# ishine/TargetDiarization

Hardware: AMD Instinct MI355X
Metric: real-time factor (audio-sec/wall-sec) full infer() pipe, 16kHz mono, 1/2/4/8 GPU (higher is better)
Workload: dtype f32 (split-f16 x3: fp32-accurate products from three f16 MFMA passes, fp32 accumulate); 1 GPU; BASELINE configs[3]: 1800 s synthetic conversation (two alternating speakers, 20 % overlap) = 180 x 10 s windows: MossFormer2 (90 windows per launch) -> loudness swap -> ERes2NetV2 on every 10 s window of both streams + cosine vs a target embedding -> Paraformer (SANM encoder, CIF predictor, NAR decoder, argmax tokens + timestamps) on 30 s segments of both streams -> CT-Transformer punctuation of ; windows_per_launch=90

## Files before the change

targetdiarization_amd/_lib.py:

```python
from __future__ import annotations

import ctypes as C
import os

HERE = os.path.dirname(os.path.abspath(__file__))
LIB_PATH = os.path.join(HERE, "libtdx.so")


class TdxError(RuntimeError):
    pass


class Mf2Config(C.Structure):
    _fields_ = [("num_blocks", C.c_int32), ("channels", C.c_int32), ("kernel_size", C.c_int32),
                ("num_spks", C.c_int32), ("group_size", C.c_int32), ("reserved", C.c_int32 * 3)]


class MdxConfig(C.Structure):
    _fields_ = [("num_blocks", C.c_int32), ("l", C.c_int32), ("g", C.c_int32), ("k", C.c_int32), ("bn", C.c_int32),
                ("dim_f", C.c_int32), ("dim_t", C.c_int32), ("reserved", C.c_int32)]


class WhisperConfig(C.Structure):
    _fields_ = [("n_mels", C.c_int32), ("n_audio_ctx", C.c_int32), ("d_model", C.c_int32), ("enc_heads", C.c_int32),
# ... 159 lines not shown
    "tdx_pvoc_destroy": (_i, [_vp]),
    "tdx_pvoc_prepare": (_i, [_vp, _i]),
    "tdx_pvoc_workspace_bytes": (_sz, [_vp, _i, _i, _i, C.c_long, C.c_long]),
    "tdx_pvoc_stretch": (_i, [_vp, _fp, _i, C.c_long, _vp, _vp, _vp, _i, C.c_long, _fp, _fp, _fp, _vp, _sz, _vp]),
    "tdx_pvoc_vocode": (_i, [_vp, _fp, _i, _i, _i, _vp, _vp, _vp, _i, _fp, _vp]),
    "tdx_pvoc_istft": (_i, [_vp, _fp, _i, _i, _i, C.c_long, _fp, _vp, _sz, _vp]),
    "tdx_pvoc_eq_match": (_i, [_vp, _fp, C.c_long, _fp, C.c_long, _fp, _i, _i, _i, _fp, _fp, _vp, _vp, _fp, _vp, _sz, _vp]),
    "tdx_resample_sinc_length": (C.c_long, [C.c_long, C.c_double]),
    "tdx_resample_sinc": (_i, [_fp, _i, C.c_long, C.c_double, _fp, C.c_long, _vp]),
    "tdx_spectral_workspace_bytes": (_sz, [_i, _i, _i]),
    "tdx_spectral_laplacian": (_i, [_fp, _i, _i, _i, _vp, _vp, _vp, _sz, _vp]),
    "tdx_symeig_lowest": (_i, [_vp, _i, _i, _vp, _vp, _vp, _sz, _vp]),
    "tdx_fft_workspace_bytes": (_sz, [C.c_long, _i]),
    "tdx_fft_c2c": (_i, [_fp, C.c_long, _i, _i, _fp, _vp, _sz, _vp]),
    "tdx_fft_r2c": (_i, [_fp, C.c_long, _i, _fp, _vp, _sz, _vp]),
    "tdx_fft_c2r": (_i, [_fp, C.c_long, _i, _fp, _vp, _sz, _vp]),
    "tdx_fft_band_mix_workspace_bytes": (_sz, [C.c_long]),
    "tdx_fft_band_mix": (_i, [_fp, _fp, C.c_long, C.POINTER(C.c_long), _fp, _fp, _fp, _fp, _vp, _sz, _vp]),
}


def lib():
    global _lib
    if _lib is None:
        if not os.path.exists(LIB_PATH):
            raise TdxError(f"{LIB_PATH} not found: build it with `python -m targetdiarization_amd.build` "
                           "(hipcc --offload-arch=gfx950).  There is no CPU fallback.")
        import torch
        tl = os.path.join(os.path.dirname(torch.__file__), "lib", "libamdhip64.so")
        if os.path.exists(tl):
            C.CDLL(tl, mode=C.RTLD_GLOBAL)
        l = C.CDLL(LIB_PATH)
        for name, (res, args) in SIGNATURES.items():
            fn = getattr(l, name)
            fn.restype = res
            fn.argtypes = args
        _lib = l
    return _lib


_l = C.c_long


class GemmSeg(C.Structure):
    _fields_ = [("A", _vp), ("B", _vp), ("lda", _l), ("ldb", _l), ("strideA", _l), ("strideB", _l), ("strideA2", _l), ("strideB2", _l),
                ("K", _i), ("zdiv", _i), ("kchunk", _i), ("ktotal", _i)]


class H3Seg(C.Structure):
    _fields_ = [("A", _vp), ("B", _vp), ("sa", _vp), ("sb", _vp), ("lda", _l), ("ldb", _l),
                ("strideA", _l), ("strideB", _l), ("strideA2", _l), ("strideB2", _l),
                ("strideSA", _l), ("strideSB", _l), ("strideSA2", _l), ("strideSB2", _l),
                ("sa_mul", _i), ("sb_mul", _i), ("K", _i), ("zdiv", _i), ("kchunk", _i), ("ktotal", _i), ("segk", _i),
                ("strideSeg", _l), ("a_shift", _i), ("a_period", _i), ("a_zero", _vp)]


DIAG_SIGNATURES = {
    "tdx_diag_last_error": (C.c_char_p, []),
    "tdx_h3_gemm_ex": (_i, [_i] * 4 + [C.POINTER(H3Seg)] * 2 + [_i] * 12 + [_vp, _vp, _l, _l, _i, C.POINTER(_i), _vp]),
    "tdx_h3_gemm_f32a": (_i, [_vp, _l, C.c_float, _vp, _vp, _vp] + [_i] * 8 + [_vp, _l, _i, _vp]),
    "tdx_h3_plan": (_i, [_i] * 5 + [C.POINTER(_i)] * 2),
    "tdx_h3_tile_of_block": (_i, [C.POINTER(_i), _i, _i, _i] + [C.POINTER(_i)] * 3),
    "tdx_h3_split_rows_static": (_i, [_vp, _l, _vp, _l, _i, C.c_float, _vp]),
    "tdx_h3_split_rows_long": (_i, [_vp, _l, _vp, _vp, _l, _i, _vp]),
    "tdx_h3_split_kmajor_ex": (_i, [_vp, _l, _vp, _l, _i, C.c_float, _i, _vp, _vp, _i, _i, _vp]),
    "tdx_h3_split_rows": (_i, [_vp, _l, _vp, _vp, _l, _i, _vp]),
    "tdx_h3_split_kmajor": (_i, [_vp, _l, _vp, _l, _i, C.c_float, _vp]),
    "tdx_h3_gemm_x": (_i, [_i] + [_vp] * 5 + [_i] * 3 + [_vp]),
    "tdx_h3_gemm": (_i, [_vp] * 6 + [_i] * 3 + [_vp]),
    "tdx_h3_gemm_variant": (_i, [_vp] * 6 + [_i] * 4 + [_vp]),
    "tdx_linear_variant": (_i, [_vp, _vp, _i, _i, _i, _vp, _i, _vp]),
    "tdx_linear_epi": (_i, [_vp] * 5 + [_i] * 5 + [_vp]),
    "tdx_gemm_f32": (_i, [_i] * 3 + [C.POINTER(GemmSeg)] * 2 + [_i] * 5 + [_vp, _l, _l, _i, C.POINTER(_i), _vp]),
    "tdx_gemm_f32_conv": (_i, [_vp, _l, _vp] + [_i] * 11 + [_vp, _l, _i, C.POINTER(_i), _vp]),
    "tdx_attn_gate_planes_workspace_bytes": (_sz, [_i, _i, _i]),
    "tdx_attn_gate_planes": (_i, [_vp] * 7 + [_i] * 5 + [_vp] * 5 + [_sz, _vp]),
    "tdx_diag_dft_analysis": (_i, [_i, _i, _l, _l, _l, _i, _vp]),
    "tdx_diag_dft_synthesis": (_i, [_i, _i, _l, _l, _i, _vp]),
    "tdx_diag_loader_bind": (_i, [_vp, _sz] + [_i] * 9 + [_vp, _sz, C.POINTER(_i)]),
    "tdx_test_whisper_noise": (_i, [C.c_ulonglong, C.c_ulonglong, _i, _i, _i, _vp, _vp, _vp]),
    "tdx_test_fft_workspace_bytes": (_sz, [_l, _i, _i]),
    "tdx_test_fft_passes": (_i, [_i, _i]),
    "tdx_test_fft_c2c": (_i, [_vp, _l, _i, _i, _vp, _vp, _sz, _vp, _i]),
    "tdx_fill_bench": (_i, [_i, _vp, _l, _i, _i, _vp, _vp]),
    "tdx_fill_bench2": (_i, [_i, _vp, _i, _i, _i, _vp, _vp]),
    "tdx_fill_bench3": (_i, [_vp, _l, _i, _l, _i, _i, _i, _vp, _vp]),
}
DIAG_PATH = os.path.join(HERE, "libtdx_diag.so")
_diag = None


def diag():
    global _diag
    if _diag is None:
        if not os.path.exists(DIAG_PATH):
            raise TdxError(f"{DIAG_PATH} not found: build it with `python -m targetdiarization_amd.build`")
        lib()
        l = C.CDLL(DIAG_PATH)
        for name, (res, args) in DIAG_SIGNATURES.items():
            fn = getattr(l, name)
            fn.restype = res
            fn.argtypes = args
        _diag = l
    return _diag


def check(status: int):
    if status != 0:
        raise TdxError(f"libtdx status {status}: {lib().tdx_last_error().decode()}")


class HandleGuard:

    def __init__(self, device):
        import threading
        self.device = device
        self.lock = threading.RLock()
        self._event = None
        self._ws = None

    def call(self):
        return _GuardedCall(self)

    def workspace(self, nbytes: int):
        import torch
        nbytes = max(int(nbytes), 16)
        if self._ws is None or self._ws.numel() < nbytes:
            if self._ws is not None and self._event is not None:
                self._event.synchronize()
            self._ws = None
            self._ws = torch.empty(nbytes, dtype=torch.uint8, device=self.device)
        return self._ws


class _GuardedCall:
    def __init__(self, g):
        self.g = g

    def __enter__(self):
        import torch
        g = self.g
        g.lock.acquire()
        try:
            self.stream = torch.cuda.current_stream(g.device)
            self.capturing = torch.cuda.is_current_stream_capturing()
            if g._event is not None and not self.capturing:
                self.stream.wait_event(g._event)
        except BaseException:
            g.lock.release()
            raise
        return g

    def __exit__(self, *exc):
        import torch
        g = self.g
        try:
            if not self.capturing:
                if g._event is None:
                    g._event = torch.cuda.Event()
                g._event.record(self.stream)
        finally:
            g.lock.release()
        return False


class Handle:
# ... 82 lines not shown
```

targetdiarization_amd/csrc/diag.hip:

```cpp
#include <hip/hip_runtime.h>

#include <algorithm>
#include <climits>
#include <initializer_list>
#include <string>

#include "../../include/tdx.h"
#include "../../include/tdx_test.h"
#include "dft_basis.hpp"
#include "epilogues.hpp"
#include "fft.hpp"
#include "gemm_h3f.hpp"
#include "mf2_attention.hpp"
#include "weight_pack.hpp"
#include "whisper_noise.hpp"

using namespace tdx;

namespace {
template <class Act>
int linear_epi(const float* a, const float* w, const float* bias, const float* res, float* out, int M, int Npad, int nreal, int K, hipStream_t st) {
    if (res && nreal < Npad) return linear_f32(a, K, w, M, Npad, K, EpiBiasResN<Act>{bias, res, out, Npad, nreal}, st);
    if (res) return linear_f32(a, K, w, M, Npad, K, EpiBiasRes<Act>{bias, res, out, Npad}, st);
    if (nreal < Npad) return linear_f32(a, K, w, M, Npad, K, EpiBiasActN<Act>{bias, out, Npad, nreal}, st);
    return linear_f32(a, K, w, M, Npad, K, EpiBiasAct<Act>{bias, out, Npad}, st);
}

struct EpiPlainN {
    float* out; long ld, strideZ; int nreal;
    __device__ EpiNone col(int, int) const { return EpiNone{}; }
    __device__ EpiNone row(int, int) const { return EpiNone{}; }
    __device__ void store(int z, int m, int n, float v, EpiNone, EpiNone) const {
        if (n < nreal) out[(long)z * strideZ + (long)m * ld + n] = v;
    }
};
struct EpiPlainPair {
    float* out; long ld, strideZ; int nreal, pair_off;
    __device__ EpiNone col(int, int) const { return EpiNone{}; }
    __device__ EpiNone row(int, int) const { return EpiNone{}; }
    __device__ void store2(int z, int m, int c, float v0, float v1, EpiNone, EpiNone) const {
        if (c < nreal) {
            float* o = out + (long)z * strideZ + (long)m * ld;
            o[c] = v0; o[pair_off + c] = v1;
        }
    }
};

void plan_out(const GemmArgs& g, int* plan) {
    if (plan) { plan[0] = g.map_mode; plan[1] = g.mp; plan[2] = g.gw; plan[3] = g.tiles_m; plan[4] = g.tiles_n; }
}
template <bool PAIRED, bool CONV>
void plan_of(GemmArgs g, int batches, int* plan) {
    plan_gemm<PAIRED, CONV>(g, batches);
    plan_out(g, plan);
}

const char* seg_error(const tdx_gemm_seg& s, bool a_kmajor, bool b_kmajor, int batches) {
    if (!s.A || !s.B) return "null operand";
    if (s.K < 32 || s.K % 32) return "need K >= 32, K % 32 == 0";
    if (s.lda < 1 || s.ldb < 1 || s.lda % 4 || s.ldb % 4) return "need lda % 4 == 0, ldb % 4 == 0";
    if (s.strideA < 0 || s.strideB < 0 || s.strideA2 < 0 || s.strideB2 < 0 || s.strideA % 4 || s.strideB % 4 || s.strideA2 % 4 || s.strideB2 % 4)
        return "need batch strides >= 0 and % 4 == 0 (16-byte loads)";
    if (s.zdiv < 1 || s.kchunk < 0) return "need zdiv >= 1, kchunk >= 0";
    if ((a_kmajor || b_kmajor) && (long)s.ktotal - (long)(std::min(s.zdiv, batches) - 1) * s.kchunk < 1)
        return "need ktotal - z2 * kchunk >= 1 for every z2 of a K-major operand";
    return nullptr;
}
GemmSeg seg_of(const tdx_gemm_seg& s) {
    GemmSeg r = make_seg(s.A, s.lda, s.B, s.ldb, s.K, s.strideA, s.strideB, s.ktotal);
    r.zdiv = s.zdiv; r.strideA2 = s.strideA2; r.strideB2 = s.strideB2; r.kchunk = s.kchunk; r.ktotal = s.ktotal;
    return r;
}
template <bool A_KMAJOR, bool B_KMAJOR, bool PAIRED, bool CONV, class Epi>
int run_gemm_f32(const GemmArgs& g, int batches, Epi e, int* plan, hipStream_t st) {
    plan_of<PAIRED, CONV>(g, batches, plan);
    const hipError_t r = launch_gemm<A_KMAJOR, B_KMAJOR, PAIRED, false, Epi, 0, CONV>(g, batches, e, st);
    return r == hipSuccess ? TDX_OK : tdx::fail_hip(r, __FILE__, __LINE__);
}

H3Seg h3_seg_of(const tdx_h3_seg& s) {
    H3Seg r{};
    r.A = (const unsigned char*)s.A; r.B = (const unsigned char*)s.B; r.sa = s.sa; r.sb = s.sb; r.lda = s.lda; r.ldb = s.ldb;
    r.strideA = s.strideA; r.strideB = s.strideB; r.strideA2 = s.strideA2; r.strideB2 = s.strideB2;
    r.strideSA = s.strideSA; r.strideSB = s.strideSB; r.strideSA2 = s.strideSA2; r.strideSB2 = s.strideSB2;
    r.sa_mul = s.sa_mul; r.sb_mul = s.sb_mul; r.K = s.K; r.zdiv = s.zdiv; r.kchunk = s.kchunk; r.ktotal = s.ktotal;
    r.segk = s.segk; r.strideSeg = s.strideSeg; r.a_shift = s.a_shift; r.a_period = s.a_period; r.a_zero = (const unsigned char*)s.a_zero;
    return r;
}
const char* h3_seg_error(const tdx_h3_seg& s, int form, bool first, int batches) {
    const bool twoseg = form & 4, shift_ok = first && form == 4;
    if (!s.A || !s.B || !s.sa || !s.sb) return "null operand or scale";
    if (s.K < 16 || s.K % 16) return "need K >= 16, K % 16 == 0";
    if (twoseg && s.K < 64) return "TWOSEG needs K >= 64 in both segments";
    if (s.lda < 64 || s.ldb < 64 || s.lda % 16 || s.ldb % 16) return "need lda, ldb >= 64 bytes and % 16 == 0 (16-byte loads)";
    for (long v : {s.strideA, s.strideB, s.strideA2, s.strideB2})
        if (v < 0 || v % 16) return "need operand strides >= 0 and % 16 == 0 (16-byte loads)";
// ... 446 lines not shown
    const long row0 = (long)(blockIdx.x / strips) * rows_per_block;
    const int per_row = seg / 1024;
    const int rows_per_it = 32 / per_row;
    float acc = 0.f;
    for (int it = 0; it < iters; ++it) {
        unsigned char* dst = lds + (it & 3) * 32768;
#pragma unroll
        for (int j = 0; j < 4; ++j) {
            const int i = wave * 4 + j;
            const long r = row0 + ((long)it * rows_per_it + i / per_row) % rows_per_block;
            const unsigned char* g = src + r * pitch + (long)strip * seg + (i % per_row) * 1024 + lane * 16;
            __builtin_amdgcn_global_load_lds((const __attribute__((address_space(1))) void*)g,
                                             (__attribute__((address_space(3))) void*)(dst + i * 1024), 16, 0, 0);
        }
        if ((it & 1) == 1) { asm volatile("s_waitcnt vmcnt(4)" ::: "memory"); __builtin_amdgcn_s_barrier(); }
    }
    asm volatile("s_waitcnt vmcnt(0)" ::: "memory");
    __syncthreads();
    acc += reinterpret_cast<const float*>(lds)[threadIdx.x];
    if (acc == 123.456f) sink[0] = acc;
}
}
extern "C" int tdx_fill_bench3(const void* src, long pitch, int seg, long rows_per_block, int strips, int blocks, int iters, float* sink, void* stream) {
    static bool set = false;
    if (!set) { hipFuncSetAttribute(reinterpret_cast<const void*>(&fill_bench3_kernel), hipFuncAttributeMaxDynamicSharedMemorySize, 131072); set = true; }
    hipLaunchKernelGGL(fill_bench3_kernel, dim3(blocks), dim3(512), 131072, (hipStream_t)stream, (const unsigned char*)src, pitch, seg, rows_per_block, strips, iters, sink);
    return hipGetLastError() == hipSuccess ? TDX_OK : TDX_E_HIP;
}
extern "C" int tdx_fill_bench2(int mode, const void* src, int stride, int blocks, int iters, float* sink, void* stream) {
    static bool set = false;
    if (!set) {
        hipFuncSetAttribute(reinterpret_cast<const void*>(&fill_bench2_kernel<0>), hipFuncAttributeMaxDynamicSharedMemorySize, 131072);
        hipFuncSetAttribute(reinterpret_cast<const void*>(&fill_bench2_kernel<1>), hipFuncAttributeMaxDynamicSharedMemorySize, 131072);
        set = true;
    }
    if (mode == 0) hipLaunchKernelGGL(fill_bench2_kernel<0>, dim3(blocks), dim3(512), 131072, (hipStream_t)stream, (const unsigned char*)src, stride, iters, sink);
    else hipLaunchKernelGGL(fill_bench2_kernel<1>, dim3(blocks), dim3(512), 131072, (hipStream_t)stream, (const unsigned char*)src, stride, iters, sink);
    return hipGetLastError() == hipSuccess ? TDX_OK : TDX_E_HIP;
}
extern "C" int tdx_fill_bench(int mode, const void* src, long bytes_per_block, int blocks, int iters, float* sink, void* stream) {
    static bool set = false;
    if (!set) {
        hipFuncSetAttribute(reinterpret_cast<const void*>(&fill_bench_kernel<0>), hipFuncAttributeMaxDynamicSharedMemorySize, 131072);
        hipFuncSetAttribute(reinterpret_cast<const void*>(&fill_bench_kernel<1>), hipFuncAttributeMaxDynamicSharedMemorySize, 131072);
        set = true;
    }
    if (mode == 0) hipLaunchKernelGGL(fill_bench_kernel<0>, dim3(blocks), dim3(512), 131072, (hipStream_t)stream, (const unsigned char*)src, bytes_per_block, iters, sink);
    else hipLaunchKernelGGL(fill_bench_kernel<1>, dim3(blocks), dim3(512), 131072, (hipStream_t)stream, (const unsigned char*)src, bytes_per_block, iters, sink);
    return hipGetLastError() == hipSuccess ? TDX_OK : TDX_E_HIP;
}

static bool fft_tile_ok(int tile_log2) { return tile_log2 >= tdx::fft::MIN_TILE_LOG2 && tile_log2 <= tdx::fft::MAX_TILE_LOG2; }
extern "C" size_t tdx_test_fft_workspace_bytes(long n, int batch, int tile_log2) {
    if (tdx::fft::size_error(n, batch) || !fft_tile_ok(tile_log2)) return 0;
    return std::max<size_t>(tdx::fft::c2c_ws_floats(n, batch, tile_log2), 64) * sizeof(float);
}
extern "C" int tdx_test_fft_passes(int m, int tile_log2) { return m < 0 || m > 27 || !fft_tile_ok(tile_log2) ? 0 : tdx::fft::passes_of(m, tile_log2); }
extern "C" int tdx_test_fft_c2c(const float* x_dev, long n, int batch, int inverse, float* y_dev, void* ws, size_t ws_bytes, void* stream, int tile_log2) {
    if (!x_dev || !y_dev || !ws || x_dev == y_dev) return tdx::fail(TDX_E_INVALID, "tdx_test_fft_c2c: need x_dev, y_dev, ws, x_dev != y_dev");
    if (const char* e = tdx::fft::size_error(n, batch)) return tdx::fail(TDX_E_INVALID, std::string("tdx_test_fft_c2c: ") + e);
    if (!fft_tile_ok(tile_log2)) return tdx::fail(TDX_E_INVALID, "tdx_test_fft_c2c: need 4 <= tile_log2 <= 12");
    if (ws_bytes < tdx_test_fft_workspace_bytes(n, batch, tile_log2)) return tdx::fail(TDX_E_INVALID, "tdx_test_fft_c2c: workspace too small");
    return tdx::fft::c2c(x_dev, n, batch, inverse != 0, y_dev, (float*)ws, tile_log2, (hipStream_t)stream);
}

namespace {
__global__ __launch_bounds__(256) void whisper_noise_kernel(unsigned long long seed, unsigned long long row_stream, int p, int n0, int count,
                                                             float* __restrict__ g, unsigned* __restrict__ word) {
    const int i = blockIdx.x * 256 + threadIdx.x;
    if (i >= count) return;
    const int n = n0 + i;
    const unsigned w = tdx::wh_noise_words(seed, row_stream, p, n >> 2).w[n & 3];
    word[i] = w;
    g[i] = tdx::wh_gumbel(w);
}
}
extern "C" int tdx_test_whisper_noise(unsigned long long seed, unsigned long long row_stream, int p, int n0, int count, float* g_dev, unsigned* word_dev,
                                      void* stream) {
    if (!g_dev || !word_dev || n0 < 0 || p < 0 || count < 1 || n0 > INT_MAX - count)
        return tdx::fail(TDX_E_INVALID, "tdx_test_whisper_noise: need g_dev, word_dev, n0 >= 0, p >= 0, count >= 1");
    hipLaunchKernelGGL(whisper_noise_kernel, dim3((count + 255) / 256), dim3(256), 0, (hipStream_t)stream, seed, row_stream, p, n0, count, g_dev, word_dev);
    return hipGetLastError() == hipSuccess ? TDX_OK : TDX_E_HIP;
}
```

targetdiarization_amd/csrc/paraformer.hip:

```cpp
#include <hip/hip_runtime.h>

#include <cmath>
#include <string>
#include <vector>

#include "../../include/tdx.h"
#include "gemm.hpp"
#include "gemm_x6.hpp"
#include "gemm_h3.hpp"
#include "shared_kernels.hpp"
#include "tdx_common.hpp"
#include "weight_planes.hpp"
#include "epilogues.hpp"
#include "pf_sanm.hpp"
#include "pf_timestamps.hpp"

using namespace tdx;

namespace {

constexpr int D = 512, DIN = 560, DINP = 576, FFN = 2048, H = 4, DK = 128, KS = 11;
constexpr float PF_LN_EPS = 1e-12f;



__global__ void pf_embed_kernel(const float* __restrict__ feats, const float* __restrict__ embed, PfPrompt pr, int nprompt, float* __restrict__ x, int T) {
    const int t = blockIdx.x, b = blockIdx.y, S = nprompt + T;
    const float pos = (float)(t + 1);
    const float inc = 9.210340371976184f / (float)(DIN / 2 - 1);
    const long row = (long)b * S + t;
    const float* src = t < nprompt ? embed + (long)pr.id[t] * DIN : feats + ((long)b * T + (t - nprompt)) * DIN;
    for (int c = threadIdx.x; c < DINP; c += blockDim.x) {
        float v = 0.f;
        if (c < DIN) {
            const int i = c < DIN / 2 ? c : c - DIN / 2;
            const float ang = __fmul_rn(pos, expf((float)i * (-inc)));
            v = src[c] * 22.627416997969522f + (c < DIN / 2 ? sinf(ang) : cosf(ang));
        }
        x[row * DINP + c] = v;
    }
}

__global__ __launch_bounds__(256) void pf_layernorm_kernel(const float* __restrict__ x, long ld, int C, const float* __restrict__ g,
                                                            const float* __restrict__ b, float* __restrict__ out, long ldo, int Cpad,
                                                            long M, float eps) {
    const long m = (long)blockIdx.x * 4 + (threadIdx.x >> 6);
    if (m >= M) return;
    const int lane = threadIdx.x & 63;
    const float* r = x + m * ld;
    float s = 0.f;
    for (int c = lane; c < C; c += 64) s += r[c];
    const float mean = wave_sum(s) / (float)C;
    float q = 0.f;
    for (int c = lane; c < C; c += 64) { const float d = r[c] - mean; q = fmaf(d, d, q); }
    const float rstd = 1.0f / sqrtf(wave_sum(q) / (float)C + eps);
    float* o = out + m * ldo;
    for (int c = lane; c < Cpad; c += 64) o[c] = c < C ? (r[c] - mean) * rstd * g[c] + b[c] : 0.f;
}

template <int NCH>
__global__ __launch_bounds__(256) void pf_layernorm_planes_kernel_t(const float* __restrict__ x, long ld, int C, const float* __restrict__ g,
                                                                     const float* __restrict__ b, unsigned char* __restrict__ hp,
                                                                     float* __restrict__ hs, int Cpad, long M, float eps) {
    const long m = (long)blockIdx.x * 4 + (threadIdx.x >> 6);
    if (m >= M) return;
    const int lane = threadIdx.x & 63;
    const float* r = x + m * ld;
    if (C == Cpad && (C & 511) == 0 && C / 512 <= NCH && (ld & 3) == 0) {
        const int nc = C / 512;
        float xv[NCH][8];
        float s1 = 0.f;
#pragma unroll
        for (int i = 0; i < NCH; ++i) {
            if (i < nc) {
                const f32x4 a0 = ldg4(r + (lane + 64 * i) * 8), a1 = ldg4(r + (lane + 64 * i) * 8 + 4);
#pragma unroll
                for (int j = 0; j < 4; ++j) { xv[i][j] = a0[j]; xv[i][4 + j] = a1[j]; s1 += a0[j] + a1[j]; }
            }
        }
        const float mean1 = wave_sum(s1) / (float)C;
        float q1 = 0.f;
#pragma unroll
        for (int i = 0; i < NCH; ++i)
            if (i < nc) {
#pragma unroll
                for (int j = 0; j < 8; ++j) { const float d = xv[i][j] - mean1; q1 = fmaf(d, d, q1); }
            }
        const float rstd1 = 1.0f / sqrtf(wave_sum(q1) / (float)C + eps);
        float mu1 = 0.f;
#pragma unroll
        for (int i = 0; i < NCH; ++i)
            if (i < nc) {
                const int c0 = (lane + 64 * i) * 8;
                const f32x4 g0 = ldg4(g + c0), g1 = ldg4(g + c0 + 4), b0 = ldg4(b + c0), b1 = ldg4(b + c0 + 4);
#pragma unroll
                for (int j = 0; j < 4; ++j) {
                    xv[i][j] = (xv[i][j] - mean1) * rstd1 * g0[j] + b0[j];
// ... 51 lines not shown
        for (int j = 0; j < 8; ++j) { if (lane * 8 + j >= S) v[j] = -INFINITY; mx1 = fmaxf(mx1, v[j]); }
        mx1 = wave_max(mx1);
        float s1 = 0.f;
#pragma unroll
        for (int j = 0; j < 8; ++j) { v[j] = lane * 8 + j < S ? expf(v[j] - mx1) : 0.f; s1 += v[j]; }
        const float inv1 = 1.0f / wave_sum(s1);
#pragma unroll
        for (int j = 0; j < 4; ++j) { a0[j] = v[j] * inv1; a1[j] = v[4 + j] * inv1; }
        *reinterpret_cast<f32x4*>(row + lane * 8) = a0;
        *reinterpret_cast<f32x4*>(row + lane * 8 + 4) = a1;
        return;
    }
    float mx = -INFINITY;
    for (int c = lane; c < S; c += 64) mx = fmaxf(mx, row[c]);
    mx = wave_max(mx);
    float s = 0.f;
    for (int c = lane; c < S; c += 64) { const float e = expf(row[c] - mx); row[c] = e; s += e; }
    s = wave_sum(s);
    const float inv = 1.0f / s;
    for (int c = lane; c < Sp; c += 64) row[c] = c < S ? row[c] * inv : 0.f;
}

constexpr int PF_FA_ROWS = 8, PF_FA_MAXT = 512;
constexpr long PF_FA_WORK = 1L << 21;
__global__ __launch_bounds__(256) void pf_attn_small_kernel(const float* __restrict__ q, long ldq, long sq, const float* __restrict__ k, long ldk, long sk,
                                                            const float* __restrict__ v, long ldv, long sv, float* __restrict__ out, long ldo, long so,
                                                            int Tq, int Tk, float scale) {
    __shared__ __attribute__((aligned(16))) float qs[PF_FA_ROWS][DK];
    __shared__ __attribute__((aligned(16))) float p[PF_FA_ROWS][PF_FA_MAXT];
    const int b = blockIdx.z, h = blockIdx.y, r0 = blockIdx.x * PF_FA_ROWS, tid = threadIdx.x;
    for (int i = tid; i < PF_FA_ROWS * DK; i += 256) {
        const int r = i >> 7, d = i & 127;
        qs[r][d] = q[(long)b * sq + (long)min(r0 + r, Tq - 1) * ldq + h * DK + d] * scale;
    }
    __syncthreads();
    for (int j = tid; j < Tk; j += 256) {
        const float4* kp = reinterpret_cast<const float4*>(k + (long)b * sk + (long)j * ldk + h * DK);
        float acc[PF_FA_ROWS];
#pragma unroll
        for (int r = 0; r < PF_FA_ROWS; ++r) acc[r] = 0.f;
#pragma unroll 8
        for (int d4 = 0; d4 < DK / 4; ++d4) {
            const float4 kv = kp[d4];
#pragma unroll
            for (int r = 0; r < PF_FA_ROWS; ++r) {
                const float4 qv = *reinterpret_cast<const float4*>(&qs[r][4 * d4]);
                acc[r] = fmaf(qv.x, kv.x, fmaf(qv.y, kv.y, fmaf(qv.z, kv.z, fmaf(qv.w, kv.w, acc[r]))));
            }
        }
#pragma unroll
        for (int r = 0; r < PF_FA_ROWS; ++r) p[r][j] = acc[r];
    }
    __syncthreads();
    {
        const int lane = tid & 63, w = tid >> 6;
#pragma unroll
        for (int rr = 0; rr < 2; ++rr) {
            float* row = p[2 * w + rr];
            float mx = -INFINITY;
            for (int c = lane; c < Tk; c += 64) mx = fmaxf(mx, row[c]);
            mx = wave_max(mx);
            float sum = 0.f;
            for (int c = lane; c < Tk; c += 64) { const float e = expf(row[c] - mx); row[c] = e; sum += e; }
            sum = wave_sum(sum);
            const float inv = 1.0f / sum;
            for (int c = lane; c < Tk; c += 64) row[c] *= inv;
        }
    }
    __syncthreads();
    {
        const int r = tid >> 5, d4 = tid & 31;
        const float* vp = v + (long)b * sv + h * DK + 4 * d4;
        float4 acc = make_float4(0.f, 0.f, 0.f, 0.f);
#pragma unroll 8
        for (int j = 0; j < Tk; ++j) {
            const float4 vv = *reinterpret_cast<const float4*>(vp + (long)j * ldv);
            const float pr = p[r][j];
            acc.x = fmaf(pr, vv.x, acc.x); acc.y = fmaf(pr, vv.y, acc.y); acc.z = fmaf(pr, vv.z, acc.z); acc.w = fmaf(pr, vv.w, acc.w);
        }
        if (r0 + r < Tq) *reinterpret_cast<float4*>(out + (long)b * so + (long)(r0 + r) * ldo + h * DK + 4 * d4) = acc;
    }
}
inline bool pf_attn_small_fits(int B, int Tq, int Tk) { return Tk <= PF_FA_MAXT && (long)B * H * Tq * Tk <= PF_FA_WORK; }

struct EpiBiasReluPl8 { const float* b; unsigned char* P; float* sc; long segs;
    __device__ float col(int, int n) const { return b[n]; }
    __device__ EpiNone row(int, int) const { return EpiNone{}; }
    __device__ float val(int, int, int, float v, EpiNone, float c) const { return fmaxf(v + c, 0.f); }
    __device__ tdx::H3PlOut plout(int) const { return tdx::H3PlOut{P, 4L * FFN, sc, nullptr, segs}; }
    __device__ long prow(int, int m) const { return m; } };
struct EpiScores { float* sc; int Sp; float scale;
    __device__ EpiNone col(int, int) const { return EpiNone{}; }
    __device__ EpiNone row(int, int) const { return EpiNone{}; }
    __device__ void store(int z, int m, int n, float v, EpiNone, EpiNone) const { sc[((long)z * Sp + m) * Sp + n] = v * scale; } };
struct EpiCtx { float* ctx; int S;
    __device__ EpiNone col(int, int) const { return EpiNone{}; }
    __device__ EpiNone row(int, int) const { return EpiNone{}; }
    __device__ void store(int z, int m, int n, float v, EpiNone, EpiNone) const {
        ctx[((long)(z / H) * S + m) * D + (z % H) * DK + n] = v; } };

constexpr long PF_SPLITK_ROWS = 512;
constexpr size_t PF_SLAB = (size_t)PF_SPLITK_ROWS * 8192;
enum { RK_BIAS = 0, RK_BIAS_RELU = 1, RK_BIAS_RES = 2, RK_OUTPROJ = 3, RK_STORE = 4 };
template <int MODE>
__global__ __launch_bounds__(256) void pf_splitk_reduce_kernel(const float* __restrict__ slab, int nsplit, long M, int N, const float* __restrict__ bias,
                                                                float* __restrict__ out, long ldo, const float* __restrict__ mem, const float* __restrict__ resid) {
    const long i4 = (long)blockIdx.x * 256 + threadIdx.x;
    if (i4 >= M * (N / 4)) return;
    const long m = i4 / (N / 4);
    const int n = (int)(i4 - m * (N / 4)) * 4;
    float4 v = make_float4(0.f, 0.f, 0.f, 0.f);
    for (int z = 0; z < nsplit; ++z) {
        const float4 p = *reinterpret_cast<const float4*>(slab + ((long)z * M + m) * N + n);
        v.x += p.x; v.y += p.y; v.z += p.z; v.w += p.w;
    }
    if (MODE != RK_STORE) { const float4 b = *reinterpret_cast<const float4*>(bias + n); v.x += b.x; v.y += b.y; v.z += b.z; v.w += b.w; }
    if (MODE == RK_BIAS_RELU) { v.x = fmaxf(v.x, 0.f); v.y = fmaxf(v.y, 0.f); v.z = fmaxf(v.z, 0.f); v.w = fmaxf(v.w, 0.f); }
    float4* o = reinterpret_cast<float4*>(out + m * ldo + n);
    if (MODE == RK_BIAS_RES) { const float4 x = *o; v.x += x.x; v.y += x.y; v.z += x.z; v.w += x.w; }
    if (MODE == RK_OUTPROJ) {
        float4 a = *reinterpret_cast<const float4*>(mem + m * D + n);
        if (resid) { const float4 r = *reinterpret_cast<const float4*>(resid + m * D + n); a.x += r.x; a.y += r.y; a.z += r.z; a.w += r.w; }
        v.x += a.x; v.y += a.y; v.z += a.z; v.w += a.w;
    }
    *o = v;
}
inline int pf_nsplit(long M, int K) {
    if (M > PF_SPLITK_ROWS || K < 512) return 1;
    int ns = K / 128; if (ns > 16) ns = 16;
    while (ns > 1 && (K % ns || (K / ns) % 32)) --ns;
    return ns;
}
inline int pf_launch_fsmn(const Conv17Args& a, int T, int B, hipStream_t st) {
    const dim3 block(128, 2);
    const long rows = (long)T * B;
    if (rows >= 512L * 256) hipLaunchKernelGGL((conv17_kernel<0, 128, KS>), dim3(1, (T + 2 * 128 - 1) / (2 * 128), B), block, 0, st, a);
    else if (rows >= 512L * 32) hipLaunchKernelGGL((conv17_kernel<0, 16, KS>), dim3(1, (T + 2 * 16 - 1) / (2 * 16), B), block, 0, st, a);
    else hipLaunchKernelGGL((conv17_kernel<0, 4, KS>), dim3(1, (T + 2 * 4 - 1) / (2 * 4), B), block, 0, st, a);
    LAUNCH_CHECK();
    return TDX_OK;
}

template <int MODE>
int lin3_splitk(const unsigned char* Ap, const float* As, const H3W& W, int M, int N, int K, int nsplit, float* slab, const float* bias, float* out,
                long ldo, const float* mem, const float* resid, hipStream_t st) {
    const int Kc = K / nsplit;
    H3Args g{};
    g.seg[0] = h3_seg(Ap, As, 4L * K, W.p, W.s, 4L * K, Kc);
    g.seg[0].strideA = 4L * Kc; g.seg[0].strideB = 4L * Kc;
    g.nseg = 1; g.M = M; g.N = N;
    if (launch_gemm_h3<false>(g, nsplit, EpiStoreZ{slab, (long)N, (long)M * N}, st) != hipSuccess) return tdx::fail_hip(hipGetLastError(), __FILE__, __LINE__);
    hipLaunchKernelGGL((pf_splitk_reduce_kernel<MODE>), dim3((unsigned)(((long)M * (N / 4) + 255) / 256)), dim3(256), 0, st, slab, nsplit, (long)M, N, bias, out, ldo, mem, resid);
    LAUNCH_CHECK();
    return TDX_OK;
}

}

struct tdx_pfenc {
    int device = 0;
    int L = 0; tdx::DevBuf dev, dev_planes; std::vector<PfLayer> layers; const float *ang = nullptr, *anb = nullptr;
};

extern "C" {

int tdx_pfenc_create(int num_blocks, const void* blob, size_t blob_bytes, int device, tdx_pfenc** out) {
// ... 15 lines not shown
    return TDX_OK;
}

int tdx_pfenc_destroy(tdx_pfenc* h) {
    delete h;
    return TDX_OK;
}

size_t tdx_pfenc_workspace_bytes(const tdx_pfenc* h, int B, int T) {
    if (!h || B < 1 || T < 1) return 0;
    return pf_work_floats(B, T) * sizeof(float);
}

double tdx_pfenc_flops(const tdx_pfenc* h, int B, int T) {
    if (!h) return 0.0;
    const double M = (double)B * T, S = T;
    double per = 2.0 * M * (3.0 * D * D + D * D + 2.0 * D * FFN) + 2.0 * B * H * (2.0 * S * S * DK) + 2.0 * M * D * KS;
    double first = 2.0 * M * 3.0 * D * (DIN - D);
    return h->L * per + first;
}

int tdx_pfenc_forward(tdx_pfenc* h, const float* feats, const int* lens_host, int B, int T, float* out, void* ws_, size_t ws_bytes,
                      void* stream) {
    if (!h || !feats || !out || !ws_ || B < 1 || T < 1) return tdx::fail(TDX_E_INVALID, "tdx_pfenc_forward: bad argument");
    if (lens_host) for (int b = 0; b < B; ++b) if (lens_host[b] != T)
        return tdx::fail(TDX_E_INVALID, "tdx_pfenc_forward: bucket segments by length (all lens must equal T)");
    if (ws_bytes < tdx_pfenc_workspace_bytes(h, B, T)) return tdx::fail(TDX_E_WORKSPACE, "tdx_pfenc_forward: workspace too small");
    tdx::DeviceGuard guard(h->device);
    if (guard.err != hipSuccess) return tdx::fail_hip(guard.err, __FILE__, __LINE__);
    hipStream_t st = (hipStream_t)stream;
    const long M = (long)B * T;
    const PfWork k = pf_carve((float*)ws_, M, B, T);
    float* x = k.x;
    TRY(pf_embed_rows(feats, nullptr, PfPrompt{}, 0, k.xin, B, T, st));
    TRY(pf_run_layers(h->layers.data(), h->L, true, x, k, B, T, st));
    return pf_layernorm_rows(x, h->ang, h->anb, out, M, st);
}

}


size_t pf_work_floats(size_t B, size_t T) {
    const size_t M = B * T, Sp = (T + 127) / 128 * 128;
    return al(M * D) + al(M * DINP) + al(M * DINP) + al((M + 128) * 3 * D) + al(B * H * Sp * Sp) + al(M * D) + al(M * D) +
           al(M * FFN) + al(M * FFN) + al(M) + 8 * al(M) + PF_SLAB;
}
PfWork pf_carve(float* ws, long M, int B, int T) {
    const int Sp = (T + 127) / 128 * 128;
    PfWork k;
    k.x = ws; k.xin = k.x + al(M * D); float* hbuf = k.xin + al(M * DINP); k.qkv = hbuf + al(M * DINP);
    k.sc = k.qkv + al((M + 128) * 3 * D); k.ctx = k.sc + al((size_t)B * H * Sp * Sp); k.mem = k.ctx + al(M * D);
    k.ffn = k.mem + al(M * D);
    k.hp = (unsigned char*)(k.ffn + al(M * FFN));
    k.hs = (float*)k.hp + al(M * FFN);
    k.hs8 = k.hs + al(M);
    k.slab = k.hs8 + 8 * al(M);
    return k;
}
void pf_stage_layer(tdx::Loader& ld, const std::string& p, bool wide, PfLayer& w) {
    const int din = wide ? DIN : D, dinp = wide ? DINP : D;
    ld.push_rows_padded(w.Wqkv, ld.get(p + "self_attn.linear_q_k_v.weight", (size_t)3 * D * din), 3 * D, din, dinp);
    ld.push(w.bqkv, ld.get(p + "self_attn.linear_q_k_v.bias", 3 * D), 3 * D);
    ld.push_tapmajor(w.fsmnT, ld.get(p + "self_attn.fsmn_block.weight", (size_t)D * KS), D, KS);
    ld.push(w.Wo, ld.get(p + "self_attn.linear_out.weight", (size_t)D * D), (size_t)D * D);
    ld.push(w.bo, ld.get(p + "self_attn.linear_out.bias", D), D);
    ld.push(w.W1, ld.get(p + "feed_forward.w_1.weight", (size_t)FFN * D), (size_t)FFN * D);
    ld.push(w.b1, ld.get(p + "feed_forward.w_1.bias", FFN), FFN);
    ld.push(w.W2, ld.get(p + "feed_forward.w_2.weight", (size_t)D * FFN), (size_t)D * FFN);
    ld.push(w.b2, ld.get(p + "feed_forward.w_2.bias", D), D);
    ld.push(w.n1g, ld.get(p + "norm1.weight", din), din); ld.push(w.n1b, ld.get(p + "norm1.bias", din), din);
    ld.push(w.n2g, ld.get(p + "norm2.weight", D), D); ld.push(w.n2b, ld.get(p + "norm2.bias", D), D);
}
void pf_queue_planes(bool wide, PfLayer& w, std::vector<tdx::PlaneJob>& jobs) {
    auto job = [&](const float* m, int N, int K, H3W& dst) { jobs.push_back({m, N, K, &dst.p, &dst.s}); };
    job(w.Wqkv, 3 * D, wide ? DINP : D, w.hqkv); job(w.Wo, D, D, w.ho);
    job(w.W1, FFN, D, w.h1); job(w.W2, D, FFN, w.h2);
}
int pf_run_layers(const PfLayer* layers, int n, bool wide_first, float* x, const PfWork& k, int B, int T, hipStream_t st) {
    const long M = (long)B * T;
    const int Sp = (T + 127) / 128 * 128;
    float *xin = k.xin, *qkv = k.qkv, *sc = k.sc, *ctx = k.ctx, *mem = k.mem, *ffn = k.ffn, *hs = k.hs, *hs8 = k.hs8, *slab = k.slab;
    unsigned char* hp = k.hp;
    const dim3 rows4((unsigned)((M + 3) / 4));
    for (int l = 0; l < n; ++l) {
        const PfLayer& w = layers[l];
        const bool first = wide_first && l == 0;
        const float* xl = first ? xin : x;
        const long ldx = first ? DINP : D;
        const int din = first ? DIN : D, dinp = first ? DINP : D;
        hipLaunchKernelGGL(pf_layernorm_planes_kernel, rows4, dim3(256), 0, st, xl, ldx, din, w.n1g, w.n1b, hp, hs, dinp, M, PF_LN_EPS);
        LAUNCH_CHECK();
        if (const int ns = pf_nsplit(M, dinp); ns > 1)
            TRY(lin3_splitk<RK_BIAS>(hp, hs, w.hqkv, (int)M, 3 * D, dinp, ns, slab, w.bqkv, qkv, 3 * D, nullptr, nullptr, st));
        else
            TRY(linear_h3(hp, hs, (int)M, w.hqkv, 3 * D, dinp, EpiBiasAct<>{w.bqkv, qkv, 3 * D}, st));
        {
            Conv17Args a{};
            a.in = qkv; a.ld_in = 3 * D; a.col0 = 2 * D; a.wT = w.fsmnT; a.C = D; a.out = mem; a.ld_out = D; a.S = T; a.Sp = T;
            TRY(pf_launch_fsmn(a, T, B, st));
        }
        if (pf_attn_small_fits(B, T, T)) {
            hipLaunchKernelGGL(pf_attn_small_kernel, dim3((T + PF_FA_ROWS - 1) / PF_FA_ROWS, H, B), dim3(256), 0, st, qkv, 3L * D, (long)T * 3 * D, qkv + D, 3L * D,
                               (long)T * 3 * D, qkv + 2 * D, 3L * D, (long)T * 3 * D, ctx, (long)D, (long)T * D, T, T, 0.08838834764831845f);
            LAUNCH_CHECK();
        } else {
        {
            GemmSeg s = make_seg(qkv, 3 * D, qkv + D, 3 * D, DK, (long)T * 3 * D, (long)T * 3 * D);
            s.zdiv = H; s.strideA2 = DK; s.strideB2 = DK;
            GemmArgs g = make_args(T, Sp, s);
            if (launch_gemm<false, false, false, false>(g, B * H, EpiScores{sc, Sp, 0.08838834764831845f}, st) != hipSuccess)
                return tdx::fail_hip(hipGetLastError(), __FILE__, __LINE__);
        }
        hipLaunchKernelGGL(pf_softmax_kernel, dim3((T + 3) / 4, B * H), dim3(256), 0, st, sc, T, Sp);
        LAUNCH_CHECK();
        {
            GemmSeg s = make_seg(sc, Sp, qkv + 2 * D, 3 * D, Sp, (long)Sp * Sp, 0, T);
            s.zdiv = 1;
            GemmArgs g = make_args(T, DK, s);
            g.seg[0].zdiv = H; g.seg[0].strideA = (long)H * Sp * Sp; g.seg[0].strideA2 = (long)Sp * Sp;
            g.seg[0].strideB = (long)T * 3 * D; g.seg[0].strideB2 = DK; g.seg[0].kchunk = 0; g.seg[0].ktotal = T;
            if (launch_gemm<false, true, false, false>(g, B * H, EpiCtx{ctx, T}, st) != hipSuccess)
                return tdx::fail_hip(hipGetLastError(), __FILE__, __LINE__);
        }
        }
        if (launch_h3_split_rows(ctx, D, hp, hs, M, D, st) != hipSuccess) return tdx::fail_hip(hipGetLastError(), __FILE__, __LINE__);
        const int ns512 = pf_nsplit(M, D), ns2048 = pf_nsplit(M, FFN);
        if (ns512 > 1) TRY(lin3_splitk<RK_OUTPROJ>(hp, hs, w.ho, (int)M, D, D, ns512, slab, w.bo, x, D, mem, first ? nullptr : x, st));
        else TRY(linear_h3(hp, hs, (int)M, w.ho, D, D, EpiBiasRes2<>{w.bo, mem, first ? nullptr : x, x, D}, st));
        hipLaunchKernelGGL(pf_layernorm_planes_kernel, rows4, dim3(256), 0, st, x, (long)D, D, w.n2g, w.n2b, hp, hs, D, M, PF_LN_EPS);
        LAUNCH_CHECK();
        if (ns512 <= 1 && ns2048 <= 1) {
            TRY(linear_h3(hp, hs, (int)M, w.h1, FFN, D, EpiBiasReluPl8{w.b1, reinterpret_cast<unsigned char*>(ffn), hs8, (long)al(M)}, st));
            H3Args g{};
            g.seg[0] = h3_seg(ffn, hs8, 4L * FFN, w.h2.p, w.h2.s, 4L * FFN, FFN);
            g.seg[0].segk = 256; g.seg[0].strideSeg = (long)al(M);
            g.nseg = 1; g.M = (int)M; g.N = D;
            if (launch_gemm_h3<false>(g, 1, EpiBiasRes<>{w.b2, x, x, D}, st) != hipSuccess) return tdx::fail_hip(hipGetLastError(), __FILE__, __LINE__);
        } else {
        if (ns512 > 1) TRY(lin3_splitk<RK_BIAS_RELU>(hp, hs, w.h1, (int)M, FFN, D, ns512, slab, w.b1, ffn, FFN, nullptr, nullptr, st));
        else TRY(linear_h3(hp, hs, (int)M, w.h1, FFN, D, EpiBiasAct<ActRelu>{w.b1, ffn, FFN}, st));
        if (launch_h3_split_rows(ffn, FFN, hp, hs, M, FFN, st) != hipSuccess) return tdx::fail_hip(hipGetLastError(), __FILE__, __LINE__);
        if (ns2048 > 1) TRY(lin3_splitk<RK_BIAS_RES>(hp, hs, w.h2, (int)M, D, FFN, ns2048, slab, w.b2, x, D, nullptr, nullptr, st));
        else TRY(linear_h3(hp, hs, (int)M, w.h2, D, FFN, EpiBiasRes<>{w.b2, x, x, D}, st));
        }
    }
    return TDX_OK;
}
int pf_embed_rows(const float* feats, const float* embed, PfPrompt pr, int nprompt, float* x, int B, int T, hipStream_t st) {
    hipLaunchKernelGGL(pf_embed_kernel, dim3(nprompt + T, B), dim3(256), 0, st, feats, embed, pr, nprompt, x, T);
    LAUNCH_CHECK();
    return TDX_OK;
}
int pf_layernorm_rows(const float* x, const float* g, const float* b, float* out, long M, hipStream_t st) {
    hipLaunchKernelGGL(pf_layernorm_kernel, dim3((unsigned)((M + 3) / 4)), dim3(256), 0, st, x, (long)D, D, g, b, out, (long)D, D, M, PF_LN_EPS);
    LAUNCH_CHECK();
    return TDX_OK;
}


namespace {

constexpr float CIF_THRESHOLD = 1.0f, CIF_TAIL = 0.45f;

__global__ __launch_bounds__(256) void pf_im2col3_planes_kernel(const float* __restrict__ enc, unsigned char* __restrict__ hp, float* __restrict__ hs,
                                                                 long M, int T) {
    const long m = (long)blockIdx.x * 4 + (threadIdx.x >> 6);
    if (m >= M) return;
    const int lane = threadIdx.x & 63;
    const int t = (int)(m % T);
    float v[3][8];
    float mu = 0.f;
#pragma unroll
    for (int i = 0; i < 3; ++i) {
        const int ch = lane + 64 * i;
        const int tap = ch >> 6, c0 = (ch & 63) * 8;
        const int ts = t + tap - 1;
        const bool ok = ts >= 0 && ts < T;
        const float* r = enc + (m + tap - 1) * D + c0;
#pragma unroll
        for (int j = 0; j < 8; ++j) { v[i][j] = ok ? r[j] : 0.f; mu = fmaxf(mu, fabsf(v[i][j])); }
    }
    float inv;
    const float sc = h3_row_scale(wave_max(mu), inv);
#pragma unroll
    for (int i = 0; i < 3; ++i) h3_store_chunk(hp + m * (4L * 3 * D) + (lane + 64 * i) * 32, v[i], sc);
    if (lane == 0) hs[m] = inv;
}
// ... 374 lines not shown
```

Before: 511.0 audio-s/s.

## Fuse Paraformer self-attention into a single split-f16 MFMA kernel

Adds a fused attention kernel for the Paraformer SANM encoder that handles QK^T, softmax and PV in one launch. Scores are held in registers for up to 512 keys, and K/V tiles are double-buffered in shared memory as hi/lo f16 planes with per-row scaling. It replaces the previous score GEMM, softmax kernel and context GEMM when T is at most 512 and the small-attention path does not apply. This removes the score buffer round-trip through global memory and two extra launches. The costs are heavy register pressure (32 f32x4 score tiles per lane), a 512-thread block with one wave per 16 queries, and an environment variable to switch it off.

```diff
diff --git a/targetdiarization_amd/_lib.py b/targetdiarization_amd/_lib.py
--- a/targetdiarization_amd/_lib.py
+++ b/targetdiarization_amd/_lib.py
@@ -265,6 +265,7 @@
     "tdx_test_fft_workspace_bytes": (_sz, [_l, _i, _i]),
     "tdx_test_fft_passes": (_i, [_i, _i]),
     "tdx_test_fft_c2c": (_i, [_vp, _l, _i, _i, _vp, _vp, _sz, _vp, _i]),
+    "tdx_test_pf_attention": (_i, [_vp, _i, _i, _vp, _vp]),
     "tdx_fill_bench": (_i, [_i, _vp, _l, _i, _i, _vp, _vp]),
     "tdx_fill_bench2": (_i, [_i, _vp, _i, _i, _i, _vp, _vp]),
     "tdx_fill_bench3": (_i, [_vp, _l, _i, _l, _i, _i, _i, _vp, _vp]),
diff --git a/targetdiarization_amd/csrc/diag.hip b/targetdiarization_amd/csrc/diag.hip
--- a/targetdiarization_amd/csrc/diag.hip
+++ b/targetdiarization_amd/csrc/diag.hip
@@ -12,6 +12,7 @@
 #include "fft.hpp"
 #include "gemm_h3f.hpp"
 #include "mf2_attention.hpp"
+#include "pf_attention.hpp"
 #include "weight_pack.hpp"
 #include "whisper_noise.hpp"
 
@@ -624,3 +625,9 @@
     hipLaunchKernelGGL(whisper_noise_kernel, dim3((count + 255) / 256), dim3(256), 0, (hipStream_t)stream, seed, row_stream, p, n0, count, g_dev, word_dev);
     return hipGetLastError() == hipSuccess ? TDX_OK : TDX_E_HIP;
 }
+
+extern "C" int tdx_test_pf_attention(const float* qkv_dev, int B, int T, float* ctx_dev, void* stream) {
+    if (!qkv_dev || !ctx_dev || B < 1 || T < 1 || T > PFA_MAXT || B > 65535)
+        return tdx::fail(TDX_E_INVALID, "tdx_test_pf_attention: need qkv_dev, ctx_dev, 1 <= B <= 65535, 1 <= T <= 512");
+    return launch_pf_attention(qkv_dev, 1536, 512, 4, B, T, ctx_dev, (hipStream_t)stream) == hipSuccess ? TDX_OK : TDX_E_HIP;
+}
diff --git a/targetdiarization_amd/csrc/paraformer.hip b/targetdiarization_amd/csrc/paraformer.hip
--- a/targetdiarization_amd/csrc/paraformer.hip
+++ b/targetdiarization_amd/csrc/paraformer.hip
@@ -13,6 +13,7 @@
 #include "weight_planes.hpp"
 #include "epilogues.hpp"
 #include "pf_sanm.hpp"
+#include "pf_attention.hpp"
 #include "pf_timestamps.hpp"
 
 using namespace tdx;
@@ -230,6 +231,11 @@
     }
 }
 inline bool pf_attn_small_fits(int B, int Tq, int Tk) { return Tk <= PF_FA_MAXT && (long)B * H * Tq * Tk <= PF_FA_WORK; }
+inline bool pf_attn_fused_fits(int B, int T) { return T <= PFA_MAXT && !pf_attn_small_fits(B, T, T); }
+inline bool pf_attn_fused_enabled() {
+    const char* e = getenv("TDX_PF_ATTN");
+    return !(e && e[0] == '0' && e[1] == 0);
+}
 
 struct EpiBiasReluPl8 { const float* b; unsigned char* P; float* sc; long segs;
     __device__ float col(int, int n) const { return b[n]; }
@@ -411,6 +417,7 @@
     float *xin = k.xin, *qkv = k.qkv, *sc = k.sc, *ctx = k.ctx, *mem = k.mem, *ffn = k.ffn, *hs = k.hs, *hs8 = k.hs8, *slab = k.slab;
     unsigned char* hp = k.hp;
     const dim3 rows4((unsigned)((M + 3) / 4));
+    const bool fused = pf_attn_fused_fits(B, T) && pf_attn_fused_enabled();
     for (int l = 0; l < n; ++l) {
         const PfLayer& w = layers[l];
         const bool first = wide_first && l == 0;
@@ -432,6 +439,8 @@
             hipLaunchKernelGGL(pf_attn_small_kernel, dim3((T + PF_FA_ROWS - 1) / PF_FA_ROWS, H, B), dim3(256), 0, st, qkv, 3L * D, (long)T * 3 * D, qkv + D, 3L * D,
                                (long)T * 3 * D, qkv + 2 * D, 3L * D, (long)T * 3 * D, ctx, (long)D, (long)T * D, T, T, 0.08838834764831845f);
             LAUNCH_CHECK();
+        } else if (fused) {
+            if (launch_pf_attention(qkv, 3L * D, D, H, B, T, ctx, st) != hipSuccess) return tdx::fail_hip(hipGetLastError(), __FILE__, __LINE__);
         } else {
         {
             GemmSeg s = make_seg(qkv, 3 * D, qkv + D, 3 * D, DK, (long)T * 3 * D, (long)T * 3 * D);
diff --git a/targetdiarization_amd/csrc/pf_attention.hpp b/targetdiarization_amd/csrc/pf_attention.hpp
--- /dev/null
+++ b/targetdiarization_amd/csrc/pf_attention.hpp
@@ -0,0 +1,240 @@
+#pragma once
+#include <hip/hip_runtime.h>
+
+#include <type_traits>
+
+#include "gemm_h3.hpp"
+
+namespace tdx {
+
+constexpr int PFA_MAXT = 512;
+constexpr int PFA_DK = 128, PFA_QB = 128, PFA_KB = 32, PFA_THREADS = 512;
+constexpr int PFA_KPITCH = 528, PFA_VPITCH = 144;
+constexpr int PFA_STAGE = PFA_DK * PFA_VPITCH;
+static_assert(PFA_KB * PFA_KPITCH <= PFA_STAGE, "K image fits a stage");
+constexpr int PFA_NKB = PFA_MAXT / PFA_KB;
+
+struct PfaRawKV { f32x4 k0, k1, v0, v1; };
+struct PfaRawV { float v[2][4]; };
+
+__device__ __forceinline__ void pfa_split8(const float* x, float s, f16x8& hi, f16x8& lo) {
+#pragma unroll
+    for (int i = 0; i < 8; ++i) {
+        const float xs = x[i] * s;
+        const _Float16 a = (_Float16)xs;
+        hi[i] = a;
+        lo[i] = (_Float16)(xs - (float)a);
+    }
+}
+
+__global__ __launch_bounds__(PFA_THREADS) void pf_attention_kernel(const float* __restrict__ qkv, long ld, int D, int T, float* __restrict__ ctx,
+                                                                   float score_scale) {
+    __shared__ __attribute__((aligned(16))) unsigned char stage[2][PFA_STAGE];
+    __shared__ __attribute__((aligned(16))) float kinv[2][PFA_KB];
+    __shared__ __attribute__((aligned(16))) float vmul[PFA_MAXT];
+    __shared__ __attribute__((aligned(16))) float vinv[PFA_MAXT];
+    const int tid = threadIdx.x, lane = tid & 63, wave = tid >> 6;
+    const int n = lane & 15, g = lane >> 4;
+    const int b = blockIdx.z, h = blockIdx.y, q0 = blockIdx.x * PFA_QB + wave * 16;
+    const int nkb = (T + PFA_KB - 1) / PFA_KB;
+    const bool wave_on = q0 < T;
+    const float* base = qkv + (long)b * T * ld + h * PFA_DK;
+
+    const int srow = tid >> 4, sc8 = tid & 15;
+    auto load_kv = [&](int j, PfaRawKV& r) {
+        const float* p = base + (long)min(min(j, nkb - 1) * PFA_KB + srow, T - 1) * ld + D + sc8 * 8;
+        r.k0 = ldg4(p); r.k1 = ldg4(p + 4);
+        r.v0 = ldg4(p + D); r.v1 = ldg4(p + D + 4);
+    };
+    auto stage_k = [&](int j, const PfaRawKV& r) {
+        const int key = j * PFA_KB + srow;
+        const float x[8] = {r.k0[0], r.k0[1], r.k0[2], r.k0[3], r.k1[0], r.k1[1], r.k1[2], r.k1[3]};
+        float mk = 0.f, mv = 0.f;
+#pragma unroll
+        for (int i = 0; i < 4; ++i) {
+            mk = fmaxf(mk, fmaxf(fabsf(r.k0[i]), fabsf(r.k1[i])));
+            mv = fmaxf(mv, fmaxf(fabsf(r.v0[i]), fabsf(r.v1[i])));
+        }
+        mk = h3_row16_max(mk);
+        mv = h3_row16_max(mv);
+        if (key >= T) mv = 0.f;
+        float ki, vi;
+        const float ks = h3_row_scale(mk, ki), vs = h3_row_scale(mv, vi);
+        f16x8 hi, lo;
+        pfa_split8(x, ks, hi, lo);
+        unsigned char* d = stage[j & 1] + srow * PFA_KPITCH + sc8 * 16;
+        *reinterpret_cast<f16x8*>(d) = hi;
+        *reinterpret_cast<f16x8*>(d + 256) = lo;
+        if (sc8 == 0 && key < PFA_MAXT) { kinv[j & 1][srow] = ki; vmul[key] = vs; vinv[key] = vi; }
+    };
+    auto load_v = [&](int j, PfaRawV& r) {
+#pragma unroll
+        for (int i = 0; i < 4; ++i) {
+            const int key = min(j, nkb - 1) * PFA_KB + 4 * wave + i;
+            const float* p = base + (long)min(key, T - 1) * ld + 2 * D + lane;
+            r.v[0][i] = p[0]; r.v[1][i] = p[64];
+        }
+    };
+    auto stage_v = [&](int j, const PfaRawV& r) {
+        const int key0 = j * PFA_KB + 4 * wave;
+        const f32x4 s4 = *reinterpret_cast<const f32x4*>(&vmul[min(key0, PFA_MAXT - 4)]);
+#pragma unroll
+        for (int c = 0; c < 2; ++c) {
+            f16x4 hi, lo;
+#pragma unroll
+            for (int i = 0; i < 4; ++i) {
+                const float xs = key0 + i < T ? r.v[c][i] * s4[i] : 0.f;
+                const _Float16 a = (_Float16)xs;
+                hi[i] = a;
+                lo[i] = (_Float16)(xs - (float)a);
+            }
+            unsigned char* d = stage[j & 1] + (lane + 64 * c) * PFA_VPITCH + (wave & 3) * 16 + (wave >> 2) * 8;
+            *reinterpret_cast<f16x4*>(d) = hi;
+            *reinterpret_cast<f16x4*>(d + 64) = lo;
+        }
+    };
+
+    f16x8 qh[4], ql[4];
+    float qc;
+    {
+        const float* p = base + (long)min(q0 + n, T - 1) * ld + 8 * g;
+        float x[4][8];
+        float mq = 0.f;
+#pragma unroll
+        for (int ks = 0; ks < 4; ++ks) {
+            const f32x4 a = ldg4(p + 32 * ks), c = ldg4(p + 32 * ks + 4);
+#pragma unroll
+            for (int i = 0; i < 4; ++i) { x[ks][i] = a[i]; x[ks][4 + i] = c[i]; mq = fmaxf(mq, fmaxf(fabsf(a[i]), fabsf(c[i]))); }
+        }
+        mq = fmaxf(mq, __shfl_xor(mq, 16, 64));
+        mq = fmaxf(mq, __shfl_xor(mq, 32, 64));
+        float qi;
+        const float qs = h3_row_scale(mq, qi);
+#pragma unroll
+        for (int ks = 0; ks < 4; ++ks) pfa_split8(x[ks], qs, qh[ks], ql[ks]);
+        qc = qi * score_scale;
+    }
+
+    f32x4 S[2 * PFA_NKB];
+#pragma unroll
+    for (int t = 0; t < 2 * PFA_NKB; ++t) S[t] = f32x4{-INFINITY, -INFINITY, -INFINITY, -INFINITY};
+    {
+        PfaRawKV R[2];
+        load_kv(0, R[0]);
+        load_kv(1, R[1]);
+        stage_k(0, R[0]);
+        load_kv(2, R[0]);
+        __syncthreads();
+        auto walk = [&](auto self, auto kbc) __attribute__((always_inline)) -> void {
+            constexpr int kb = decltype(kbc)::value;
+            if constexpr (kb < PFA_NKB) if (kb < nkb) {
+                stage_k(kb + 1, R[(kb + 1) & 1]);
+                load_kv(kb + 3, R[(kb + 1) & 1]);
+                if (wave_on) {
+                    const unsigned char* st = stage[kb & 1] + n * PFA_KPITCH + g * 16;
+#pragma unroll
+                    for (int tile = 0; tile < 2; ++tile) {
+                        f32x4 acc = {0.f, 0.f, 0.f, 0.f};
+#pragma unroll
+                        for (int ks = 0; ks < 4; ++ks) {
+                            const f16x8 ah = *reinterpret_cast<const f16x8*>(st + tile * 16 * PFA_KPITCH + ks * 64);
+                            const f16x8 al = *reinterpret_cast<const f16x8*>(st + tile * 16 * PFA_KPITCH + ks * 64 + 256);
+                            acc = __builtin_amdgcn_mfma_f32_16x16x32_f16(ah, ql[ks], acc, 0, 0, 0);
+                            acc = __builtin_amdgcn_mfma_f32_16x16x32_f16(al, qh[ks], acc, 0, 0, 0);
+                            acc = __builtin_amdgcn_mfma_f32_16x16x32_f16(ah, qh[ks], acc, 0, 0, 0);
+                        }
+                        const f32x4 ki = *reinterpret_cast<const f32x4*>(&kinv[kb & 1][tile * 16 + 4 * g]);
+                        const int key0 = kb * PFA_KB + tile * 16 + 4 * g;
+#pragma unroll
+                        for (int r = 0; r < 4; ++r) S[2 * kb + tile][r] = key0 + r < T ? acc[r] * (ki[r] * qc) : -INFINITY;
+                    }
+                }
+                __syncthreads();
+                self(self, std::integral_constant<int, kb + 1>{});
+            }
+        };
+        walk(walk, std::integral_constant<int, 0>{});
+    }
+
+    PfaRawV V[2];
+    load_v(0, V[0]);
+    load_v(1, V[1]);
+
+    float rsum = 1.f, pinv = 1.f, ps = 1.f;
+    if (wave_on) {
+        float m = -INFINITY;
+#pragma unroll
+        for (int t = 0; t < 2 * PFA_NKB; ++t) m = fmaxf(fmaxf(m, fmaxf(S[t][0], S[t][1])), fmaxf(S[t][2], S[t][3]));
+        m = fmaxf(m, __shfl_xor(m, 16, 64));
+        m = fmaxf(m, __shfl_xor(m, 32, 64));
+        float sum = 0.f, mp = 0.f;
+#pragma unroll
+        for (int t = 0; t < 2 * PFA_NKB; ++t) {
+            if (t < 2 * nkb) {
+                const f32x4 vi = *reinterpret_cast<const f32x4*>(&vinv[t * 16 + 4 * g]);
+#pragma unroll
+                for (int r = 0; r < 4; ++r) {
+                    const float p = __builtin_amdgcn_exp2f(S[t][r] - m);
+                    sum += p;
+                    const float pv = p * vi[r];
+                    S[t][r] = pv;
+                    mp = fmaxf(mp, pv);
+                }
+            }
+        }
+        sum += __shfl_xor(sum, 16, 64);
+        sum += __shfl_xor(sum, 32, 64);
+        mp = fmaxf(mp, __shfl_xor(mp, 16, 64));
+        mp = fmaxf(mp, __shfl_xor(mp, 32, 64));
+        ps = h3_row_scale(mp, pinv);
+        rsum = 1.0f / sum;
+    }
+
+    f32x4 O[8];
+#pragma unroll
+    for (int dt = 0; dt < 8; ++dt) O[dt] = f32x4{0.f, 0.f, 0.f, 0.f};
+    stage_v(0, V[0]);
+    load_v(2, V[0]);
+    __syncthreads();
+    auto walk2 = [&](auto self, auto kbc) __attribute__((always_inline)) -> void {
+        constexpr int kb = decltype(kbc)::value;
+        if constexpr (kb < PFA_NKB) if (kb < nkb) {
+            stage_v(kb + 1, V[(kb + 1) & 1]);
+            load_v(kb + 3, V[(kb + 1) & 1]);
+            if (wave_on) {
+                float x[8];
+#pragma unroll
+                for (int r = 0; r < 4; ++r) { x[r] = S[2 * kb][r]; x[4 + r] = S[2 * kb + 1][r]; }
+                f16x8 bh, bl;
+                pfa_split8(x, ps, bh, bl);
+                const unsigned char* st = stage[kb & 1] + n * PFA_VPITCH + g * 16;
+#pragma unroll
+                for (int dt = 0; dt < 8; ++dt) {
+                    const f16x8 vh = *reinterpret_cast<const f16x8*>(st + dt * 16 * PFA_VPITCH);
+                    const f16x8 vl = *reinterpret_cast<const f16x8*>(st + dt * 16 * PFA_VPITCH + 64);
+                    O[dt] = __builtin_amdgcn_mfma_f32_16x16x32_f16(vh, bl, O[dt], 0, 0, 0);
+                    O[dt] = __builtin_amdgcn_mfma_f32_16x16x32_f16(vl, bh, O[dt], 0, 0, 0);
+                    O[dt] = __builtin_amdgcn_mfma_f32_16x16x32_f16(vh, bh, O[dt], 0, 0, 0);
+                }
+            }
+            __syncthreads();
+            self(self, std::integral_constant<int, kb + 1>{});
+        }
+    };
+    walk2(walk2, std::integral_constant<int, 0>{});
+
+    if (wave_on && q0 + n < T) {
+        const float f = pinv * rsum;
+        float* o = ctx + ((long)b * T + q0 + n) * D + h * PFA_DK + 4 * g;
+#pragma unroll
+        for (int dt = 0; dt < 8; ++dt) *reinterpret_cast<f32x4*>(o + 16 * dt) = O[dt] * f;
+    }
+}
+
+inline hipError_t launch_pf_attention(const float* qkv, long ld, int D, int H, int B, int T, float* ctx, hipStream_t st) {
+    hipLaunchKernelGGL(pf_attention_kernel, dim3((T + PFA_QB - 1) / PFA_QB, H, B), dim3(PFA_THREADS), 0, st, qkv, ld, D, T, ctx,
+                       0.08838834764831845f * 1.4426950408889634f);
+    return hipGetLastError();
+}
+
+}
```

Result: no change. 513.3 audio-s/s (median of 6 runs) (+0.4%).
